# Arbol-Project/dcdf

Measured on AMD Instinct MI355X. Metric: raster cells/s encoded (Snapshot+Log build), higher is better.
Workload: dtype int32; 1 GPU; configs[2]: 4096x4096x365 i32 raster, seed 0xDCDF0003, tiled into 3072 [<=32,256,256] chunks; 3072 of them on this GPU; workload_key=config2/i32/n3072/w1, chunks_total=3072, chunks_on_rank0=3072, cells_total=6123683840, k=2, device=gfx950:sramecc+:xnack- AMD Radeon Graphics, 256 CUs, failed_tiles_rank0=0, encoded_bytes_rank0=4115239087, snapshots_rank0=3072, bytes_verified_vs_oracle=0, parallelism=chunks sharded over 1 GPU(s), no data-path collective

## Files before the change

dcdf_amd/csrc/k2r_capi_encode.hip:

```cpp
#include <algorithm>
#include <atomic>
#include <condition_variable>
#include <cstdio>
#include <cstdlib>
#include <cstring>
#include <deque>
#include <memory>
#include <mutex>
#include <new>
#include <thread>
#include <vector>

#include <sched.h>

#include <cstring>
#include <queue>

#include "k2r_launch.h"
#include "k2r_runtime.h"

using namespace k2r;

namespace k2r {

// ... 463 lines not shown
    if (std::getenv("K2R_PROFILE_PRINT")) {
        uint64_t acc[NPROF] = {0};
        for (size_t i = 0; i < n; i++)
            for (int k = 0; k < NPROF; k++) acc[k] += e->results[i].prof[k];
        uint64_t tot = 0;
        for (int k = 0; k < NPROF; k++) tot += acc[k];
        static const char* names[NPROF] = {"p1 load+analysis", "p2 top", "p3 own/top nodes", "reduce4", "clear+hdr",
                                           "emit C snapshot", "emit C/Q log", "T/eqB bitmaps", "Lmax dac | V0,M0 bitmaps", "Lmin dac | zero bitmaps",
                                           "emit pass A", "emit pass B/I", "sizes+heuristic", "winner scan", "byte-1 pass A", "fast: phase 1",
                                           "fast: wait p1", "fast: top+plan", "fast: copy-out", "fast: bitmaps"};
        for (int k = 0; k < NPROF; k++)
            std::fprintf(stderr, "k2r-prof %-18s %14llu cyc %5.1f%%\n", names[k], (unsigned long long)acc[k],
                         tot ? 100.0 * (double)acc[k] / (double)tot : 0.0);
#ifdef K2R_PROFILE
        {
            static uint64_t w[16][NPROF][2];
            std::memset(w, 0, sizeof(w));
            for (size_t i = 0; i < n; i++)
                for (int v = 0; v < 16; v++)
                    for (int k = 0; k < NPROF; k++) {
                        w[v][k][0] += e->results[i].pw[v][k][0];
                        w[v][k][1] += e->results[i].pw[v][k][1];
                    }
            int nw = 0;
            for (int v = 0; v < 16; v++) {
                uint64_t t = 0;
                for (int k = 0; k < NPROF; k++) t += w[v][k][0] + w[v][k][1];
                if (t) nw = v + 1;
            }
            uint64_t insts = 0;
            for (size_t i = 0; i < n; i++) insts += e->results[i].snapshots + e->results[i].logs;
            double all = 0;
            for (int k = 0; k < NPROF; k++)
                for (int v = 0; v < nw; v++) all += (double)(w[v][k][0] + w[v][k][1]);
            all /= nw ? nw : 1;
            std::fprintf(stderr, "k2r-pw %d waves, %llu chunk-instants, %.0f cycles per chunk-instant and wave (work + wait)\n", nw,
                         (unsigned long long)insts, insts ? all / (double)insts : 0.0);
            std::fprintf(stderr, "k2r-pw %-24s %9s %9s %9s %9s %7s   (cycles per chunk-instant)\n", "phase", "work-mean", "work-max", "work-w0",
                         "wait-mean", "share");
            for (int k = 0; k < NPROF; k++) {
                double mean = 0, mx = 0, wait = 0;
                for (int v = 0; v < nw; v++) {
                    mean += (double)w[v][k][0];
                    wait += (double)w[v][k][1];
                    mx = std::max(mx, (double)w[v][k][0]);
                }
                if (mean + wait == 0) continue;
                mean /= nw;
                wait /= nw;
                const double d = insts ? (double)insts : 1.0;
                std::fprintf(stderr, "k2r-pw %-24s %9.0f %9.0f %9.0f %9.0f %6.1f%%\n", names[k], mean / d, mx / d, (double)w[0][k][0] / d, wait / d,
                             all ? 100.0 * (mean + wait) / all : 0.0);
            }
        }
#endif
        std::vector<double> per;
        uint64_t logs = 0, stash = 0;
        for (size_t i = 0; i < n; i++) {
            uint64_t t = 0;
            for (int k = 0; k < NPROF; k++) t += e->results[i].prof[k];
            const uint32_t ni = e->results[i].snapshots + e->results[i].logs;
            if (ni) per.push_back((double)t / ni);
            logs += e->results[i].logs;
            stash += e->results[i].stash_logs;
        }
        std::sort(per.begin(), per.end());
        if (!per.empty()) {
            double sum = 0;
            for (double x : per) sum += x;
            std::fprintf(stderr, "k2r-prof cycles/instant per tile: min %.0f p50 %.0f mean %.0f p90 %.0f p99 %.0f max %.0f | logs %llu from stash %llu\n",
                         per.front(), per[per.size() / 2], sum / per.size(), per[per.size() * 9 / 10], per[per.size() * 99 / 100],
                         per.back(), (unsigned long long)logs, (unsigned long long)stash);
        }
    }
    for (size_t i = 0; i < n; i++)
        if (e->results[i].status == ST_INTERNAL) {
            const uint32_t* d = e->results[i].dbg;
            std::fprintf(stderr, "dcdf_k2r: internal guard tripped on tile %zu: guard bitmask=0x%08x (bit = kGuard* in k2r_encode.h)\n",
                         i, d[0]);
        }
    for (int pass = 0; pass < 2; pass++) {
    std::vector<std::vector<uint32_t>> again(e->classes.size());
    bool any = false, unsplit = false;
    for (size_t ci = 0; ci < e->classes.size(); ci++)
        for (uint32_t ti : e->class_tiles[ci])
            if (e->results[ti].status == ST_OUT_CAPACITY || e->results[ti].status == ST_RESPLIT) {
                if (e->results[ti].status == ST_OUT_CAPACITY) {
                    const dcdf_tile_desc& t = e->desc[ti];
                    const uint64_t cap = 6 + (uint64_t)t.instants * (1 + worst_instant_bytes((uint32_t)e->classes[ci].log2s));
                    std::unique_ptr<DevBuf> b(new DevBuf());
                    K2R_HIP(b->alloc(cap));
                    e->args[ti].out = b->as<uint8_t>();
                    e->args[ti].out_cap = cap;
                    e->retry_slots.push_back(std::move(b));
                }
                const bool was_split = e->args[ti].inst_end != 0;
                e->args[ti].inst_end = 0;
                e->args[ti].shared_flag = nullptr;
                e->args[ti].shared_cmp = nullptr;
                unsplit = unsplit || was_split;
                K2R_HIP(hipMemcpy(e->d_args.as<TileArgs>() + ti, &e->args[ti], sizeof(TileArgs), hipMemcpyHostToDevice));
                again[ci].push_back(ti);
                any = true;
            }
    if (any) {
        rc = run_classes(e, &again, nullptr);
// ... 619 lines not shown
```

dcdf_amd/csrc/k2r_encode.h:

```cpp
#pragma once
#include "k2r_exec.h"


#ifndef K2R_DIAG_SKIP
#define K2R_DIAG_SKIP 0
#endif

namespace k2r {

template <int LOG2S>
struct EncCfg {
    static_assert(LOG2S >= 3 && LOG2S <= 8, "kernel body written for sidelen 8..256 (the library dispatches 16..256)");
    static constexpr int H = LOG2S;
    static constexpr int S = 1 << LOG2S;
    static constexpr int NBLK = 1 << (2 * (LOG2S - 3));
    static constexpr int NT = NBLK;
    static constexpr int NW = NT < 64 ? 1 : NT / 64;
    static constexpr int NTOP = ((1 << (2 * (H - 2))) - 1) / 3;
    static constexpr int NTOPX = NTOP - (1 << (2 * (H - 3)));
    static constexpr int TBW = (NTOPX + 31) / 32 + 1;
    static constexpr int MAXV = ((1 << (2 * (H + 1))) - 1) / 3;
    static constexpr int MAXT = ((1 << (2 * H)) - 1) / 3;
    static constexpr int WV = (MAXV + 31) / 32;
    static constexpr int WT = (MAXT + 31) / 32;
    static constexpr int top_off(int h) { return ((1 << (2 * (H - 2))) - (1 << (2 * (H - h + 1)))) / 3; }
};

struct EncRegs {
    uint32_t d2[4];
    uint32_t flags;
    uint32_t u2;
    uint32_t sc[MAX_SCAN_FIELDS];
    uint64_t pf_lo;
    uint32_t pf_l2;
    uint32_t pa[5];
#ifdef K2R_REGCOPY
    uint32_t cw[32];
#endif
};

K2R_HD uint32_t unpackI(int h, uint64_t lo, uint64_t top) {
    switch (h) {
        case 1: return (uint32_t)(lo & 0xffffu);
        case 2: return (uint32_t)((lo >> 16) & 0x3fffu);
        case 3: return (uint32_t)((lo >> 30) & 0xfffu);
        case 4: return (uint32_t)(top & 0x3ffu);
        case 5: return (uint32_t)((top >> 10) & 0xffu);
        case 6: return (uint32_t)((top >> 18) & 0x3fu);
        case 7: return (uint32_t)((top >> 24) & 0xfu);
        case 8: return (uint32_t)((top >> 28) & 0x3u);
    }
    return 0;
}
K2R_HD uint64_t packTop(int h) {
    switch (h) {
        case 4: return 1ull;
        case 5: return 1ull << 10;
        case 6: return 1ull << 18;
        case 7: return 1ull << 24;
        case 8: return 1ull << 28;
    }
    return 0;
}

struct Cls {
    uint32_t c1 = 0, c2 = 0, c3 = 0;
    K2R_HD void add(uint32_t zz, bool on) {
        c1 += (on && zz > 0xffu) ? 1u : 0u;
        c2 += (on && zz > 0xffffu) ? 1u : 0u;
        c3 += (on && zz > 0xffffffu) ? 1u : 0u;
    }
    K2R_HD void add4(uint32_t z0, uint32_t z1, uint32_t z2, uint32_t z3, bool on) {
        if (on && ((z0 | z1 | z2 | z3) > 0xffu)) {
            add(z0, true);
            add(z1, true);
            add(z2, true);
            add(z3, true);
        }
// ... 418 lines not shown
    uint32_t offZ[C::H + 2];
    uint32_t LT, N0, M0;
    K2R_HD void from_counts(const uint32_t* ni) {
        constexpr int H = C::H;
#pragma unroll
        for (int h = 1; h <= H; h++) Ni[h] = ni[h];
        finish();
    }
    K2R_HD void from(uint64_t lo, uint64_t top) {
        constexpr int H = C::H;
#pragma unroll
        for (int h = 1; h <= H; h++) Ni[h] = unpackI(h, lo, top);
        finish();
    }
    K2R_HD void finish() {
        constexpr int H = C::H;
        Ni[H + 1] = 0;
        uint32_t v = 0, i = 0, z = 0;
#pragma unroll
        for (int h = H; h >= 0; h--) {
            uint32_t nv = (h == H) ? 1u : 4u * Ni[h + 1];
            offV[h] = v;
            offI[h] = i;
            offZ[h] = z;
            v += nv;
            if (h >= 1) {
                i += Ni[h];
                z += nv - Ni[h];
            }
        }
        N0 = v;
        LT = offV[0];
        M0 = i;
    }
};

template <class C>
struct InstPlan {
    Totals<C> T[2];
    DacLayout V[2], M[2];
    uint32_t need;
    uint32_t narrow;
    uint32_t log_size, snap_lb, eq_off;
    uint32_t as_snapshot, use_stash, isize;
    uint32_t lngV[3], lngM[3];
};

template <class C>
struct EncPool {
    static constexpr int POOL_L1 = 4 * C::NBLK;
    static constexpr int POOL_BMV1 = 12 * C::NBLK;
    static constexpr int POOL_PREFV = POOL_BMV1 + C::WV + 1;
#ifdef K2R_PROFILE
    static constexpr int POOLFILL = 1828 - 16 * NPROF * 4;
#else
    static constexpr int POOLFILL = 1828;
#endif
    static constexpr int POOLW = POOL_PREFV + C::WV + 2 + (C::H == 8 ? POOLFILL : 0);
    static constexpr int CAPI_REC = (POOLW * 53 / 100) / 5;
    static constexpr int CAPQ_REC = (POOLW - 5 * CAPI_REC) / 3;
    static constexpr int QBASE = 5 * CAPI_REC;
    static constexpr int OVI_WORDS = 5 * 4 * C::NBLK;
    static constexpr int OVQ_WORDS = 3 * 16 * C::NBLK;
};

template <class C>
struct EncShared : EncPool<C> {
    using EncPool<C>::POOL_L1;
    using EncPool<C>::POOL_BMV1;
    using EncPool<C>::POOL_PREFV;
    using EncPool<C>::POOLW;
    int32_t tmin[C::NTOP], tmax[C::NTOP], smin[C::NTOP], smax[C::NTOP], diff[C::NTOP];
    uint32_t eq[C::NTOP];
    uint32_t pool[EncPool<C>::POOLW];
    uint32_t bmT[C::WT + 1], bmE[C::WT + 1];
    uint32_t bmV0[C::WV + 1];
    uint32_t bmM[2][C::WT + 1];
    uint32_t prefM[C::WT + 2];
    uint32_t wsum[C::NW][MAX_SCAN_FIELDS];
    uint32_t tot[MAX_SCAN_FIELDS];
    K2R_HD uint32_t* L2() { return pool; }
    K2R_HD uint16_t* L1() { return (uint16_t*)(pool + POOL_L1); }
    K2R_HD uint32_t* bmV1() { return pool + POOL_BMV1; }
    K2R_HD uint32_t* prefV() { return pool + POOL_PREFV; }
    static constexpr int PREFTOP = 48;
    uint32_t prefTopV[PREFTOP + 1];
    uint32_t pfx[3][C::NBLK];
    uint32_t lq[C::NBLK][2];
    uint32_t li[C::NBLK];
    uint32_t tbS[C::TBW], tbL[C::TBW];
    uint32_t tbP[C::TBW + 1];
    uint32_t ttR[C::H + 2];
    uint32_t nlistV, nlistM;
    uint32_t stI, stQ;
    InstPlan<C> pl;
    int32_t err;
    uint32_t work;
    uint32_t fault[6];
    uint64_t prof[NPROF], prof_last;
#ifdef K2R_PROFILE
    uint64_t pw[16][NPROF][2];
#endif
};

template <class EX>
K2R_HD bool guard_ok(EX& ex, bool ok, uint32_t code, uint32_t inst, uint32_t tid, uint32_t value, uint32_t limit) {
    ex.gfail |= ok ? 0u : (1u << (code & 31u));
    (void)inst; (void)tid; (void)value; (void)limit;
    return ok;
}
template <bool UNIFORM_SPAN = true, class EX>
K2R_HD uint32_t guard_pos(EX& ex, uint32_t pos, uint32_t span, uint32_t limit, uint32_t code) {
#if defined(__HIP_DEVICE_COMPILE__) && !defined(K2R_GUARD_FULL)
    int32_t r;
    if (UNIFORM_SPAN) asm("v_med3_i32 %0, %1, 0, %2" : "=v"(r) : "v"((int32_t)pos), "s"((int32_t)limit - (int32_t)span));
    else asm("v_med3_i32 %0, %1, 0, %2" : "=v"(r) : "v"((int32_t)pos), "v"((int32_t)limit - (int32_t)span));
    (void)ex; (void)code;
    return (uint32_t)r;
#else
    const bool ok = pos + span <= limit;
    ex.gfail |= ok ? 0u : (1u << (code & 31u));
    return ok ? pos : 0u;
#endif
}
template <class EX>
K2R_HD void guard_flush(EX& ex) {
    if (ex.gfail) {
        ex.lds_or(&ex.sh.fault[0], ex.gfail);
        ex.gfail = 0;
    }
}
enum : uint32_t {
    kGuardVPos = 0, kGuardVSlot = 1, kGuardMPos = 2, kGuardMSlot = 3, kGuardTOwn = 4, kGuardEOwn = 5, kGuardTRun1 = 6,
    kGuardTRun2 = 7, kGuardE2 = 8, kGuardE1 = 9, kGuardListPos = 10, kGuardListRank = 14, kGuardList2 = 18, kGuardList1 = 19,
};

template <class EX>
K2R_HD void bm_set(EX& ex, uint32_t* bm, uint32_t p) {
    ex.lds_or(&bm[p >> 5], 0x80000000u >> (p & 31));
}
template <class EX>
K2R_HD void bm_or_run(EX& ex, uint32_t* bm, uint32_t p, uint32_t len, uint32_t bits) {
    if (len == 0 || bits == 0) return;
    const uint64_t v = (uint64_t)bits << (64 - len);
    const uint32_t sh = p & 31;
    const uint64_t w = v >> sh;
    const uint32_t hi = (uint32_t)(w >> 32), lo = (uint32_t)w;
// ... 284 lines not shown
template <class C, bool PADDED, int VEC, class EX>
K2R_HD void encode_chunk(EX& ex, const TileArgs& ta, TileResult* res, uint64_t* listV, uint64_t* listM, uint32_t* scmp, uint32_t* ovf) {
    constexpr int H = C::H;
    constexpr int NT = C::NT;
    auto& sh = ex.sh;
    using SH = EncShared<C>;
    static_assert(!(PADDED && VEC != 0), "vector loads need an unpadded tile");
    const uint32_t stash_cap = ta.stash_words != 0 ? ta.stash_words : 0xffffffffu;
    uint32_t* const ovI = ovf;
    uint32_t* const ovQ = ovf + SH::OVI_WORDS;

    uint8_t* const out = ta.out;
    const uint64_t cap = ta.out_cap;

    auto blk_origin = [&](int tid, uint32_t& r0, uint32_t& c0) {
        uint32_t br, bc;
        morton_decode((uint32_t)tid, br, bc);
        r0 = br * 8;
        c0 = bc * 8;
#if defined(__HIP_DEVICE_COMPILE__)
        asm volatile("" : "+v"(r0), "+v"(c0));
#endif
    };
    auto inval = [&](uint32_t r, uint32_t c) -> bool { return PADDED && (r >= ta.rows || c >= ta.cols); };
    auto top_inval = [&](int h, uint32_t j) -> bool {
        if (!PADDED) return false;
        uint32_t br, bc;
        morton_decode(j, br, bc);
        return inval(br << h, bc << h);
    };

    const uint32_t i_begin = ta.inst_begin, i_end = ta.inst_end != 0 ? ta.inst_end : ta.instants;
    const bool cont = i_begin > 0;
    const bool head = !cont && ta.shared_flag != nullptr;
    bool published = false;
    uint32_t* cmp = scmp;
    constexpr uint32_t NO_HDR = 0xffffffffu;
    uint32_t carry = 0;
    uint32_t off = cont ? 0u : 6u;
    uint32_t n_blocks = 0;
    uint32_t blk_hdr = cont ? NO_HDR : 6u;
    uint32_t blk_count = 0;
    uint32_t s_idx = 0;
    bool s_cmp = false;
    int32_t s_base = 0;
    uint32_t n_snap = 0, n_log = 0, n_stash = 0;
    int32_t status = ST_OK;

    ex.par([&](int tid, EncRegs&) {
        if (tid == 0) {
            sh.err = 0;
            sh.stI = 0;
            sh.stQ = 0;
            for (int i = 0; i < 6; i++) sh.fault[i] = 0;
            for (int i = 0; i < NPROF; i++) sh.prof[i] = 0;
            if (cap >= 6 && !cont) {
                out[0] = (uint8_t)ta.dtype;
                out[1] = (uint8_t)ta.fbits;
            }
        }
    });
    if (cap < 7 && !cont) status = ST_OUT_CAPACITY;
#ifdef K2R_PROFILE
    if (!EX::kSim) {
        ex.par([&](int tid, EncRegs&) {
            if (tid == 0) sh.prof_last = clock64();
            if ((tid & 63) == 0)
                for (int k = 0; k < NPROF; k++) sh.pw[tid >> 6][k][0] = sh.pw[tid >> 6][k][1] = 0;
        });
        ex.pw_start();
    }
#endif

#ifdef K2R_REGCOPY
    constexpr bool kRegCopy = !PADDED;
#else
    constexpr bool kRegCopy = false;
#endif
    [[maybe_unused]] auto lean_node = [&](uint32_t ltid, int p, uint32_t& B, uint32_t& j) {
        if (EX::kSim) {
            B = ltid;
            j = (uint32_t)p;
        } else {
            constexpr uint32_t NTW = NT < 64 ? NT : 64, BPP = NTW / 4;
            const uint32_t lane = ltid & 63u;
            B = (ltid & ~63u) + BPP * (uint32_t)p + (lane >> 2);
            j = lane & 3u;
        }
    };
    auto compact_pass = [&](uint32_t from, bool to_global) {
        if (kRegCopy) {
#ifdef K2R_REGCOPY
            ex.par_nosync([&](int tid, EncRegs& r) {
                const uint32_t ltid = opaque((uint32_t)tid);
                int32_t lerr = 0;
#pragma unroll
                for (int p = 0; p < 4; p++) {
                    uint32_t B, j, br, bc;
                    lean_node(ltid, p, B, j);
                    morton_decode(4u * B + j, br, bc);
                    int32_t t16[16];
                    load_sub16<false, VEC>(ta, from, 4u * br, 4u * bc, 0, t16, lerr);
#pragma unroll
                    for (int q = 0; q < 2; q++)
#pragma unroll
                        for (int c = 0; c < 4; c++)
// ... 684 lines not shown
        };
        auto log_vmax = [&](int h, uint32_t j) -> int32_t {
            const int a = C::top_off(h) + (int)j;
            return top_inval(h, j) ? 0 : sh.tmax[a] - sh.smax[a];
        };
        auto log_vmin = [&](int h, uint32_t j) -> int32_t {
            const int a = C::top_off(h) + (int)j;
            return sh.tmin[a] - sh.smin[a];
        };

        auto top_decode = [&](uint32_t n, int& h, uint32_t& j) {
            h = 4;
#pragma unroll
            for (int k = 4; k < H; k++)
                if (n >= (uint32_t)(C::top_off(k + 1) - C::NBLK)) h = k + 1;
            j = n - (uint32_t)(C::top_off(h) - C::NBLK);
        };
        auto tbit = [&](int h, uint32_t j) -> uint32_t { return (uint32_t)(C::top_off(h) - C::NBLK) + j; };

        ex.par_nosync([&](int tid, EncRegs& r) {
            uint32_t sI3 = 0, lI3 = 0;
            uint32_t wide = (r.flags >> 28) & 1u;
            Cls lMax, lMin;
            uint32_t sTop = 0, lTop = 0;
            auto node = [&](int h, uint32_t j) {
                if (PS(h, j)) {
                    if (h == 3) sI3 = 1;
                    else {
                        ex.lds_or(&sh.tbS[tbit(h, j) >> 5], 1u << (tbit(h, j) & 31));
                        sTop += (uint32_t)packTop(h);
                    }
                }
                if (have_s) {
                    const bool visL = (h == H) ? true : PL(h + 1, j >> 2);
                    const bool pL = PL(h, j);
                    const int32_t vx = log_vmax(h, j), vn = log_vmin(h, j);
                    lMax.add1(vx, visL);
                    lMin.add1(vn, pL);
                    wide |= ((visL && (vx < -32768 || vx > 32767)) || (pL && (vn < -32768 || vn > 32767))) ? 1u : 0u;
                    if (pL) {
                        if (h == 3) lI3 = 1;
                        else {
                            ex.lds_or(&sh.tbL[tbit(h, j) >> 5], 1u << (tbit(h, j) & 31));
                            lTop += (uint32_t)packTop(h);
                        }
                    }
                }
            };
            const uint32_t wt = opaque((uint32_t)tid);
            node(3, wt);
            if (tid == 0) {
                sh.stI = 0;
                sh.stQ = 0;
            }
            if (wt < (uint32_t)C::NTOPX) {
                int h;
                uint32_t j;
                top_decode(wt, h, j);
                node(h, j);
            }
            r.sc[1] = sI3 | (lI3 << 16);
            r.sc[2] = sTop;
            r.sc[4] = lTop;
            r.sc[5] = lMax.c1 | (lMin.c1 << 16);
            r.sc[6] = wide;
            uint32_t cL0 = 0, cL1 = 0, mL1 = 0, cL2 = 0, mL2 = 0;
            if (have_s) {
                const uint32_t fl = sh.li[tid];
                cL0 = popc32(sh.lq[tid][0]) + popc32(sh.lq[tid][1]);
                cL1 = popc32(fl & 0x0f0f0f0fu);
                mL1 = popc32(fl & 0xf0f0f0f0u);
#pragma unroll
                for (int j = 0; j < 4; j++) {
                    const int32_t vx = rec16(r.d2[j] & 0xffffu), vn = rec16(r.d2[j] >> 16);
                    r.d2[j] = ((uint32_t)vx & 0xffffu) | ((uint32_t)vn << 16);
                    const bool P2L = ((r.u2 >> j) & 1u) == 0 && ((r.flags >> j) & 1u) == 0;
                    cL2 += lI3 ? lng(vx) : 0u;
                    mL2 += P2L ? lng(vn) : 0u;
                }
            }
            r.sc[7] = cL0;
            r.sc[8] = cL1 | (cL2 << 16);
            r.sc[9] = mL1 | (mL2 << 16);
        });
        ex.stamp(2);
        ex.template scan_begin<10>();
        ex.stamp(3);

        auto classes_pass = [&](const int which) {
#ifdef K2R_SIM_TRACE
            if (EX::kSim) __builtin_printf("classes_pass(%d) inst=%u\n", which, inst);
#endif
            ex.par_nosync([&](int tid, EncRegs& r) {
                uint32_t r0, c0;
                blk_origin(tid, r0, c0);
                int32_t lerr = 0;
                Cls vMax, vMin;
                auto cnode = [&](int h, uint32_t j) {
                    if (which == 0) {
                        vMax.add(zz32(snap_vmax(h, j)), (h == H) ? true : PS(h + 1, j >> 2));
                        vMin.add(zz32(snap_vmin(h, j)), PS(h, j));
                    } else {
                        vMax.add(zz32(log_vmax(h, j)), (h == H) ? true : PL(h + 1, j >> 2));
                        vMin.add(zz32(log_vmin(h, j)), PL(h, j));
                    }
                };
// ... 205 lines not shown
        }
        if (need & 2u) {
            classes_pass(0);
            plan(3);
        }
        const bool as_snapshot = ex.uni(sh.pl.as_snapshot) != 0;
        const bool use_stash = ex.uni(sh.pl.use_stash) != 0;
        const uint32_t isize = ex.uni(sh.pl.isize);
        const uint32_t log_eq_off = ex.uni(sh.pl.eq_off);
        const Totals<C>& TT = sh.pl.T[as_snapshot ? 0 : 1];
        const DacLayout& DV = sh.pl.V[as_snapshot ? 0 : 1];
        const DacLayout& DM = sh.pl.M[as_snapshot ? 0 : 1];

        uint32_t hdr_patch_off = 0, hdr_patch_val = 0;
        bool do_patch = false;
        if (as_snapshot) {
            if (have_s) {
                if (blk_hdr == NO_HDR) carry = blk_count;
                else {
                    do_patch = true;
                    hdr_patch_off = blk_hdr;
                    hdr_patch_val = blk_count;
                }
                n_blocks++;
            }
            blk_hdr = off;
            off += 1;
            blk_count = 0;
            s_idx = inst;
            n_snap++;
            const int32_t rmin = ex.uni(sh.tmin[C::top_off(H)]), rmax = ex.uni(sh.tmax[C::top_off(H)]);
            s_cmp = (int64_t)rmax - (int64_t)rmin <= 65535 && inst + 1 < ta.instants;
            s_base = rmin;
            cmp = (head && inst == 0) ? ta.shared_cmp : scmp;
        } else {
            n_log++;
        }
        if ((uint64_t)off + isize > cap) {
            status = ST_OUT_CAPACITY;
            break;
        }
        uint8_t* const io = out + off;
        n_stash += use_stash ? 1u : 0u;
        ex.stamp(12);
        ex.par([&](int tid, EncRegs& r) {
            const uint32_t pI12 = as_snapshot ? r.sc[0] : r.sc[3];
            const uint32_t pI3 = as_snapshot ? (r.sc[1] & 0xffffu) : (r.sc[1] >> 16);
            const uint32_t pL0 = r.sc[7], pL12 = r.sc[8], pM12 = r.sc[9];
            r.pf_lo = (uint64_t)pI12 | ((uint64_t)pI3 << 30);
            r.pf_l2 = (pL12 >> 16) | (pM12 & 0xffff0000u);
            sh.pfx[0][tid] = pI12;
            sh.pfx[1][tid] = pL0;
            sh.pfx[2][tid] = (pL12 & 0xffffu) | (pM12 << 16);
            if (tid <= C::TBW) {
                const uint32_t* const tbw = as_snapshot ? sh.tbS : sh.tbL;
                uint32_t run = 0;
                for (int w = 0; w < tid && w < C::TBW; w++) run += popc32(tbw[w]);
                sh.tbP[tid] = run;
            }
            if (tid == 0) {
                sh.nlistV = 0;
                sh.nlistM = 0;
                if (do_patch) out[hdr_patch_off] = (uint8_t)hdr_patch_val;
                io[0] = 2;
                store_be32(io + 1, ta.rows);
                store_be32(io + 5, ta.cols);
                store_be32(io + 9, (uint32_t)C::S);
                io[DV.bm_off[0] - 1] = (uint8_t)DV.nlev;
                io[DM.bm_off[0] - 1] = (uint8_t)DM.nlev;
                if (ta.minmax) {
                    ta.minmax[2 * inst] = sh.tmin[C::top_off(H)];
                    ta.minmax[2 * inst + 1] = sh.tmax[C::top_off(H)];
                }
            }
        });

        ex.stamp(4);
        const uint32_t nlevV = ex.uni(DV.nlev), nlevM = ex.uni(DM.nlev);
        const DacSink sinkV{io + ex.uni(DV.by_off[0]), sh.bmV0, listV, &sh.nlistV, ex.uni(DV.n[0]), ex.uni(DV.n[1]), inst, kGuardVPos,
                            io + ex.uni(DV.by_off[1]), use_stash ? sh.prefTopV : sh.prefV()};
        const DacSink sinkM{io + ex.uni(DM.by_off[0]), sh.bmM[0], listM, &sh.nlistM, ex.uni(DM.n[0]), ex.uni(DM.n[1]), inst, kGuardMPos,
                            io + ex.uni(DM.by_off[1]), sh.prefM};

        const bool snap_dyn = as_snapshot;
        const Totals<C>& TT_dyn = TT;
        auto passA = [&](auto mode_tag) {
          constexpr int MODE = decltype(mode_tag)::value;
          ex.par_nosync([&](int tid, EncRegs& r) {
            uint32_t r0, c0;
            blk_origin(tid, r0, c0);
            const uint64_t pLo = r.pf_lo;

            const bool as_snapshot = MODE == EM_P0 ? false : snap_dyn;
            const Totals<C>& TT = MODE == EM_P0 ? sh.pl.T[1] : TT_dyn;
            const uint32_t* const tb = as_snapshot ? sh.tbS : sh.tbL;
            if (MODE == EM_P0) r.pa[2] = 0;
            constexpr int GMODE = (MODE == EM_P0) ? (int)EM_ONE : MODE;
            auto enode = [&](int h, uint32_t j, const int slot) {
                const bool vis = (h == H) ? true : bit_test(tb, tbit(h + 1, j >> 2));
                if (!vis) return;
                const bool p = (h == 3) ? (as_snapshot ? PS(3, j) : PL(3, j)) : bit_test(tb, tbit(h, j));
                auto trank = [&](uint32_t b) -> uint32_t {
                    return sh.tbP[b >> 5] + popc32(tb[b >> 5] & ((1u << (b & 31u)) - 1u));
                };
                uint32_t vrank = 0;
                if (h < H) vrank = 4 * (trank(tbit(h + 1, j >> 2)) - sh.ttR[h + 1]) + (j & 3);
                const uint32_t idx = TT.offV[h] + vrank;
                const uint32_t irank = (h == 3) ? unpackI(3, pLo, 0) : trank(tbit(h, j)) - sh.ttR[h];
                const uint32_t zv = zz32(as_snapshot ? snap_vmax(h, j) : log_vmax(h, j));
                emit_val<0, MODE>(ex, sinkV, idx, zv, tid);
                if (MODE == EM_P0) {
                    r.pa[3 * slot] = idx;
                    r.pa[2] |= (zv >> 8) << (16 * slot);
                }
                if (p) {
                    bm_set(ex, sh.bmT, guard_pos(ex, idx, 1, TT.LT, kGuardTOwn));
                    const uint32_t zm = zz32(as_snapshot ? snap_vmin(h, j) : log_vmin(h, j));
                    emit_val<1, MODE>(ex, sinkM, TT.offI[h] + irank, zm, tid);
                    if (MODE == EM_P0) {
                        r.pa[3 * slot + 1] = TT.offI[h] + irank;
                        r.pa[2] |= (zm >> 8) << (16 * slot + 8);
                    }
// ... 82 lines not shown
                                smx2 = s16[i] > smx2 ? s16[i] : smx2;
                            }
                            vx = inv2 ? 0 : mx2 - smx2;
                            vn = mn2 - smn2;
                        }
                    } else {
                        vx = (int32_t)(int16_t)(r.d2[j] & 0xffffu);
                        vn = (int32_t)r.d2[j] >> 16;
                    }
                    if (as_snapshot) {
                        P2[j] = !unif2;
                        z2v[j] = zz32(vx);
                        zm2[j] = zz32(vn);
                    } else {
                        P2[j] = !unif2 && ((r.flags >> j) & 1u) == 0;
                        z2v[j] = zz32(vx);
                        zm2[j] = zz32(vn);
                        if (!P2[j]) {
                            erun = (erun << 1) | (unif2 ? 0u : 1u);
                            elen++;
                        }
                    }
                    tb2 = (tb2 << 1) | (P2[j] ? 1u : 0u);
                }
                emit4<0, GMODE>(ex, sinkV, p2, z2v[0], z2v[1], z2v[2], z2v[3], tid, sh.pl.lngV[2] + (r.pf_l2 & 0xffffu));
                bm_or_run(ex, sh.bmT, guard_pos(ex, p2, 4, TT.LT, kGuardTRun2), 4, tb2);
                if (!as_snapshot) bm_or_run(ex, sh.bmE, guard_pos<false>(ex, TT.offZ[2] + 4 * E3 - E2, elen, TT.LT - TT.M0, kGuardE2), elen, erun);
                uint32_t n2 = 0, pre = E1, lm = sh.pl.lngM[2] + (r.pf_l2 >> 16);
                const uint32_t cshift = as_snapshot ? 4u : 16u;
#pragma unroll
                for (int j = 0; j < 4; j++) {
                    if (P2[j]) {
                        emit_val<1, GMODE>(ex, sinkM, TT.offI[2] + E2 + n2, zm2[j], tid, lm);
                        lm += zm2[j] > 0xffu ? 1u : 0u;
                        if (MODE == EM_LIST)
                            sh.L2()[guard_pos(ex, E2 + n2, 1, 4 * C::NBLK, kGuardList2)] = ((uint32_t)tid << 2) | (uint32_t)j | (pre << 12);
                        n2++;
                        pre += (r.flags >> (cshift + 3 * j)) & 7u;
                    }
                }
            }
            guard_flush(ex);
        });
        };
        const uint32_t nI2 = ex.uni(TT.Ni[2]), nI1 = ex.uni(TT.Ni[1]);
        if (use_stash) {
            if (!(K2R_DIAG_SKIP & 1)) passA(EmTag<EM_P0>{});
            ex.stamp(10);
            auto passI = [&](auto ovf_tag) {
              constexpr bool OVF = decltype(ovf_tag)::value != 0;
              ex.par_nosync([&](int tid, EncRegs&) {
                const uint32_t offV1 = TT.offV[1], offZ1 = TT.offZ[1], offI1 = TT.offI[1], lt = TT.LT, ne = TT.LT - TT.M0;
                const uint32_t lv1 = sh.pl.lngV[1], lm1 = sh.pl.lngM[1];
                for (uint32_t k = (uint32_t)tid; k < nI2; k += NT) {
                    uint32_t rec[5];
                    if (!OVF || k < (uint32_t)SH::CAPI_REC) {
#pragma unroll
                        for (int i = 0; i < 5; i++) rec[i] = sh.pool[5u * k + i];
                    } else {
                        gload_words<5>(ovI + 5u * (k - (uint32_t)SH::CAPI_REC), rec);
                    }
                    const uint32_t hdr = rec[0];
                    const uint32_t own = hdr & 1023u;
                    const uint32_t pf = sh.pfx[0][own], pl = sh.pfx[2][own];
                    const uint32_t kk = ((pf >> 16) & 0x3fffu) + ((hdr >> 10) & 3u);
                    const uint32_t pre = (pf & 0xffffu) + ((hdr >> 12) & 15u);
                    const uint32_t tb1 = (hdr >> 16) & 15u, e4 = (hdr >> 20) & 15u, elen = 4u - popc32(tb1);
                    uint32_t erun = 0;
#pragma unroll
                    for (int qq = 0; qq < 4; qq++) {
                        const uint32_t t0 = ((tb1 >> (3 - qq)) & 1u) ^ 1u;
                        erun = (erun << t0) | ((e4 >> (3 - qq)) & t0);
                    }
                    const uint32_t below = sh.li[own] & ((1u << (8u * ((hdr >> 10) & 3u))) - 1u);
                    uint32_t w[4];
#pragma unroll
                    for (int qq = 0; qq < 4; qq++) w[qq] = rec[1 + qq];
                    const uint32_t p1 = offV1 + 4 * kk;
                    emit4<0, EM_ONE>(ex, sinkV, p1, zz32(rec16(w[0] & 0xffffu)), zz32(rec16(w[1] & 0xffffu)),
                                     zz32(rec16(w[2] & 0xffffu)), zz32(rec16(w[3] & 0xffffu)), tid,
                                     lv1 + (pl & 0xffffu) + popc32(below & 0x0f0f0f0fu));
                    bm_or_run(ex, sh.bmT, guard_pos(ex, p1, 4, lt, kGuardTRun1), 4, tb1);
                    bm_or_run(ex, sh.bmE, guard_pos<false>(ex, offZ1 + 4 * kk - pre, elen, ne, kGuardE1), elen, erun);
                    uint32_t n1 = 0, lm = lm1 + (pl >> 16) + popc32(below & 0xf0f0f0f0u);
#pragma unroll
                    for (int qq = 0; qq < 4; qq++) {
                        if ((tb1 >> (3 - qq)) & 1u) {
                            const uint32_t zm = zz32(rec16(w[qq] >> 16));
                            emit_val<1, EM_ONE>(ex, sinkM, offI1 + pre + n1, zm, tid, lm);
                            lm += zm > 0xffu ? 1u : 0u;
                            n1++;
                        }
                    }
                }
                guard_flush(ex);
              });
            };
            if (K2R_DIAG_SKIP & 2) {
            } else if (rec_ovf) passI(EmTag<1>{});
            else passI(EmTag<0>{});
            ex.stamp(11);
            auto passQ = [&](auto ovf_tag) {
              constexpr bool OVF = decltype(ovf_tag)::value != 0;
              ex.par([&](int tid, EncRegs&) {
                const uint32_t offV0 = TT.offV[0], lv0 = sh.pl.lngV[0];
                for (uint32_t m = (uint32_t)tid; m < nI1; m += NT) {
                    uint32_t q[3];
                    if (!OVF || m < (uint32_t)SH::CAPQ_REC) {
#pragma unroll
                        for (int i = 0; i < 3; i++) q[i] = sh.pool[SH::QBASE + 3u * m + i];
                    } else {
                        gload_words<3>(ovQ + 3u * (m - (uint32_t)SH::CAPQ_REC), q);
                    }
                    const uint32_t hdr = q[0], a = q[1], b = q[2];
                    const uint32_t own = hdr & 1023u;
                    const uint32_t ord = (hdr >> 10) & 15u;
                    const uint32_t pos = (sh.pfx[0][own] & 0xffffu) + ord;
                    const uint32_t f0 = sh.lq[own][0], f1 = sh.lq[own][1], cut = (1u << (4u * (ord & 7u))) - 1u;
                    const uint32_t before = ord < 8u ? popc32(f0 & cut) : popc32(f0) + popc32(f1 & cut);
                    emit4<0, EM_ONE>(ex, sinkV, offV0 + 4 * pos, zz32(rec16(a & 0xffffu)), zz32(rec16(a >> 16)),
                                     zz32(rec16(b & 0xffffu)), zz32(rec16(b >> 16)), tid, lv0 + sh.pfx[1][own] + before);
                }
                guard_flush(ex);
              });
            };
            if (K2R_DIAG_SKIP & 4) ex.barrier();
            else if (rec_ovf) passQ(EmTag<1>{});
            else passQ(EmTag<0>{});
            ex.stamp(6);
            {
                const uint32_t lt = ex.uni(TT.LT), m0 = ex.uni(TT.M0);
                const BmJob jobs[4] = {{sh.bmT, lt, nullptr, 0, io + 13},
                                       {sh.bmE, lt - m0, nullptr, 0, io + log_eq_off},
                                       {sh.bmV0, sinkV.n0, sh.prefTopV, SH::PREFTOP, nlevV > 0 ? io + ex.uni(DV.bm_off[0]) : nullptr},
                                       {sh.bmM[0], sinkM.n0, sh.prefM, SH::PREFTOP, nlevM > 0 ? io + ex.uni(DM.bm_off[0]) : nullptr}};
                if (!(K2R_DIAG_SKIP & 8)) bitmaps_finish<C, 4>(ex, jobs);
            }
            ex.stamp(8);
            if (nlevV > 1 || nlevM > 1) {
                if (!(K2R_DIAG_SKIP & 16)) ex.par_nosync([&](int tid, EncRegs& r) {
                    auto put = [&](const DacSink& d, uint32_t* bm0, uint32_t pos, uint32_t hi) {
                        if (hi) {
                            pos = guard_pos(ex, pos, 1, d.n0 < 32u * SH::PREFTOP ? d.n0 : 32u * SH::PREFTOP, d.code);
                            gstore8(d.plane1 + guard_pos(ex, bm_rank(bm0, d.pref, pos), 1, d.n1, d.code + 1), (uint8_t)hi);
                        }
                    };
                    const uint32_t hb = r.pa[2];
                    put(sinkV, sh.bmV0, r.pa[0], hb & 0xffu);
                    put(sinkM, sh.bmM[0], r.pa[1], (hb >> 8) & 0xffu);
                    put(sinkV, sh.bmV0, r.pa[3], (hb >> 16) & 0xffu);
                    put(sinkM, sh.bmM[0], r.pa[4], hb >> 24);
                    guard_flush(ex);
                });
                ex.stamp(14);
                if (nlevV > 1 && !(K2R_DIAG_SKIP & 32)) bitmap_write_zero<C>(ex, sinkV.n1, io + ex.uni(DV.bm_off[1]));
                if (nlevM > 1 && !(K2R_DIAG_SKIP & 32)) bitmap_write_zero<C>(ex, sinkM.n1, io + ex.uni(DM.bm_off[1]));
            }
            ex.stamp(9);
        } else {
// ... 175 lines not shown
```

dcdf_amd/csrc/k2r_exec.h:

```cpp
#pragma once
#include "k2r_common.h"

namespace k2r {

constexpr int MAX_SCAN_FIELDS = 16;

#if defined(__HIPCC__)

template <class SH, class TR, int NT>
struct GpuExec {
    SH& sh;
    TR r;
    const int tid;
    uint32_t gfail = 0;
    static constexpr int kNT = NT;
    static constexpr bool kSim = false;

    __device__ GpuExec(SH& s) : sh(s), tid((int)threadIdx.x) {}

#ifdef K2R_PROFILE
    uint64_t pw_last = 0, pw_work = 0, pw_wait = 0;
    __device__ __forceinline__ void pw_before() {
        const uint64_t t = __builtin_amdgcn_s_memtime();
        pw_work += t - pw_last;
        pw_last = t;
    }
    __device__ __forceinline__ void pw_after() {
        const uint64_t t = __builtin_amdgcn_s_memtime();
        pw_wait += t - pw_last;
        pw_last = t;
    }
    __device__ __forceinline__ void pw_start() { pw_last = __builtin_amdgcn_s_memtime(); pw_work = pw_wait = 0; }
#else
    __device__ __forceinline__ void pw_before() {}
    __device__ __forceinline__ void pw_after() {}
    __device__ __forceinline__ void pw_start() {}
#endif

    __device__ __forceinline__ void lds_barrier() {
        pw_before();
        asm volatile("s_waitcnt lgkmcnt(0)\n\ts_barrier" ::: "memory");
        pw_after();
    }
    __device__ __forceinline__ void wave_lds_fence() { asm volatile("s_waitcnt lgkmcnt(0)" ::: "memory"); }
    __device__ __forceinline__ void barrier_global() {
        pw_before();
        __syncthreads();
        pw_after();
    }

    __device__ __forceinline__ void publish(uint32_t* flag, uint32_t value, uint32_t payload) {
        __syncthreads();
        if (tid == 0) {
            __hip_atomic_store(flag + 1, payload, __ATOMIC_RELAXED, __HIP_MEMORY_SCOPE_AGENT);
            __builtin_amdgcn_fence(__ATOMIC_RELEASE, "agent");
            __hip_atomic_store(flag, value, __ATOMIC_RELAXED, __HIP_MEMORY_SCOPE_AGENT);
        }
    }
    __device__ __forceinline__ uint32_t await(const uint32_t* flag, uint32_t timeout_value) {
        if (tid == 0) {
            uint32_t v = 0;
            for (uint32_t spin = 0; spin < (1u << 22); spin++) {
                v = __hip_atomic_load(flag, __ATOMIC_RELAXED, __HIP_MEMORY_SCOPE_AGENT);
                if (v != 0) break;
                __builtin_amdgcn_s_sleep(32);
            }
            __builtin_amdgcn_fence(__ATOMIC_ACQUIRE, "agent");
            sh.err = v != 0 ? (int32_t)v : (int32_t)timeout_value;
        }
        __syncthreads();
        const uint32_t v = (uint32_t)__builtin_amdgcn_readfirstlane(sh.err);
// ... 168 lines not shown
    }
    __device__ __forceinline__ static int32_t row_min_of_quads(int32_t x) {
        int32_t y = (int32_t)row_ror<4>((uint32_t)x);
        x = x < y ? x : y;
        y = (int32_t)row_ror<8>((uint32_t)x);
        return x < y ? x : y;
    }
    __device__ __forceinline__ static int32_t row_max_of_quads(int32_t x) {
        int32_t y = (int32_t)row_ror<4>((uint32_t)x);
        x = x > y ? x : y;
        y = (int32_t)row_ror<8>((uint32_t)x);
        return x > y ? x : y;
    }
    __device__ __forceinline__ static uint32_t row_or_of_quads(uint32_t x) {
        x |= row_ror<4>(x);
        return x | row_ror<8>(x);
    }
    __device__ __forceinline__ static int32_t wave_min_of_rows(int32_t x) {
        const int32_t a = __builtin_amdgcn_readlane(x, 0), b = __builtin_amdgcn_readlane(x, 16), c = __builtin_amdgcn_readlane(x, 32),
                      d = __builtin_amdgcn_readlane(x, 48);
        const int32_t p = a < b ? a : b, q = c < d ? c : d;
        return p < q ? p : q;
    }
    __device__ __forceinline__ static int32_t wave_max_of_rows(int32_t x) {
        const int32_t a = __builtin_amdgcn_readlane(x, 0), b = __builtin_amdgcn_readlane(x, 16), c = __builtin_amdgcn_readlane(x, 32),
                      d = __builtin_amdgcn_readlane(x, 48);
        const int32_t p = a > b ? a : b, q = c > d ? c : d;
        return p > q ? p : q;
    }
    __device__ __forceinline__ static uint32_t wave_or_of_rows(uint32_t x) {
        return (uint32_t)(__builtin_amdgcn_readlane((int)x, 0) | __builtin_amdgcn_readlane((int)x, 16) | __builtin_amdgcn_readlane((int)x, 32) |
                          __builtin_amdgcn_readlane((int)x, 48));
    }
    __device__ __forceinline__ static uint32_t lane_pull(uint32_t src, uint32_t v) {
        return (uint32_t)__builtin_amdgcn_ds_bpermute((int)(src << 2), (int)v);
    }

    __device__ __forceinline__ void stash_alloc(uint32_t c, uint32_t* cntA, uint32_t* cntB, uint32_t& a, uint32_t& b, uint32_t& enda,
                                                uint32_t& endb) {
        constexpr int W = NT < 64 ? NT : 64;
        const int lane = tid & 63;
        const uint32_t incl = wave_incl_scan(c);
        const uint32_t tot = (uint32_t)__builtin_amdgcn_readlane((int)incl, W - 1);
        uint32_t ret = 0;
        if (lane < 2) ret = atomicAdd(lane == 0 ? cntA : cntB, lane == 0 ? (tot & 0xffffu) : (tot >> 16));
        const uint32_t ba = (uint32_t)__builtin_amdgcn_readlane((int)ret, 0), bb = (uint32_t)__builtin_amdgcn_readlane((int)ret, W > 1 ? 1 : 0);
        const uint32_t excl = incl - c;
        a = ba + (excl & 0xffffu);
        b = bb + (excl >> 16);
        enda = ba + (tot & 0xffffu);
        endb = bb + (tot >> 16);
    }

    __device__ __forceinline__ uint32_t lds_or_nr(uint32_t* p, uint32_t v) { atomicOr(p, v); return 0; }
    __device__ __forceinline__ uint32_t lds_or(uint32_t* p, uint32_t v) { return atomicOr(p, v); }
    __device__ __forceinline__ uint32_t lds_add(uint32_t* p, uint32_t v) { return atomicAdd(p, v); }
    __device__ __forceinline__ int32_t lds_min(int32_t* p, int32_t v) { return atomicMin(p, v); }

    template <int NF, bool TOT = true>
    __device__ __forceinline__ void scan() {
        constexpr int W = NT < 64 ? NT : 64;
        constexpr int NW = NT < 64 ? 1 : NT / 64;
        const int lane = tid & 63;
        const int wave = __builtin_amdgcn_readfirstlane(tid >> 6);
        int incl[NF];
#pragma unroll
        for (int f = 0; f < NF; f++) incl[f] = (int)r.sc[f];
        wave_incl_scan_n(incl);
        if (lane == W - 1) {
#pragma unroll
            for (int f = 0; f < NF; f++) sh.wsum[wave][f] = (uint32_t)incl[f];
        }
        lds_barrier();
        int x[NF];
#pragma unroll
        for (int f = 0; f < NF; f++) x[f] = (lane < NW) ? (int)sh.wsum[lane < NW ? lane : 0][f] : 0;
        row_incl_scan_n(x);
#pragma unroll
        for (int f = 0; f < NF; f++) {
            const uint32_t tot = (uint32_t)__builtin_amdgcn_readlane(x[f], NW - 1);
            const uint32_t base = wave == 0 ? 0u : (uint32_t)__builtin_amdgcn_readlane(x[f], wave - 1);
            r.sc[f] = base + (uint32_t)incl[f] - r.sc[f];
            if (TOT && tid == 0) sh.tot[f] = tot;
        }
        if (TOT) lds_barrier();
    }
};

#endif

#if !defined(__HIP_DEVICE_COMPILE__)
}
#include <vector>
namespace k2r {

template <class SH, class TR, int NT>
struct SimExec {
    SH& sh;
    std::vector<TR> regs;
    uint32_t gfail = 0;
    static constexpr int kNT = NT;
    static constexpr bool kSim = true;

    explicit SimExec(SH& s) : sh(s), regs(NT) {}

    template <class F>
    void par(F&& f) {
        for (int t = 0; t < NT; t++) f(t, regs[t]);
    }
    template <class F>
    void par_nosync(F&& f) {
        for (int t = 0; t < NT; t++) f(t, regs[t]);
    }
    void barrier() {}
    void wave_lds_fence() {}
    void barrier_global() {}
    void publish(uint32_t* flag, uint32_t value, uint32_t payload) {
        flag[1] = payload;
        flag[0] = value;
    }
    uint32_t await(const uint32_t* flag, uint32_t timeout_value) { return flag[0] != 0 ? flag[0] : timeout_value; }
    uint32_t flag_payload(const uint32_t* flag) { return flag[1]; }
    void stamp(int) {}
    template <class T>
    T uni(T v) const { return v; }
    template <int NF, int F0 = 0>
    void reduce() {
        for (int f = F0; f < F0 + NF; f++) {
            uint32_t run = 0;
            for (int t = 0; t < NT; t++) run += regs[t].sc[f];
            sh.tot[f] = run;
        }
    }

    template <int NF>
    void scan_begin() {
        scan<NF, true>();
    }
    static constexpr int planner() { return 0; }
    uint32_t lane_value(uint32_t v, int) const { return v; }
    template <int NF>
    void scan_finish(uint32_t (&t)[NF]) {
        for (int f = 0; f < NF; f++) t[f] = sh.tot[f];
    }


    void stash_alloc(uint32_t c, uint32_t* cntA, uint32_t* cntB, uint32_t& a, uint32_t& b, uint32_t& enda, uint32_t& endb) {
        a = *cntA;
        b = *cntB;
        *cntA += c & 0xffffu;
        *cntB += c >> 16;
        enda = *cntA;
        endb = *cntB;
    }
    uint32_t lds_or_nr(uint32_t* p, uint32_t v) {
        *p |= v;
        return 0;
    }
    uint32_t lds_or(uint32_t* p, uint32_t v) {
        uint32_t o = *p;
        *p = o | v;
        return o;
    }
    uint32_t lds_add(uint32_t* p, uint32_t v) {
        uint32_t o = *p;
        *p = o + v;
        return o;
    }
    int32_t lds_min(int32_t* p, int32_t v) {
        int32_t o = *p;
        if (v < o) *p = v;
        return o;
    }

    template <int NF, bool TOT = true>
    void scan() {
        for (int f = 0; f < NF; f++) {
            uint32_t run = 0;
            for (int t = 0; t < NT; t++) {
                const uint32_t v = regs[t].sc[f];
                regs[t].sc[f] = run;
                run += v;
            }
            sh.tot[f] = run;
        }
    }
};
#endif

}
```

Measured before the change: 552.4 billion cells/s.

## Balance per-wave work with dynamic record claiming and rotated single-thread tasks

Replaces the static strided loops over I and Q records with wave-granular dynamic work claiming through an LDS atomic counter, so waves that finish early pick up more records. Moves the single-thread tbP prefix and header writes onto threads in different waves chosen by a rotation, and computes the tbP prefix sequentially in one thread instead of one thread per word. It also adds per-wave profiling tables to the host report. The atomic claiming adds one LDS atomic per wave iteration, and the pool shrinks by two words to make room for the counters.

```diff
diff --git a/dcdf_amd/csrc/k2r_capi_encode.hip b/dcdf_amd/csrc/k2r_capi_encode.hip
--- a/dcdf_amd/csrc/k2r_capi_encode.hip
+++ b/dcdf_amd/csrc/k2r_capi_encode.hip
@@ -539,6 +539,45 @@
                 std::fprintf(stderr, "k2r-pw %-24s %9.0f %9.0f %9.0f %9.0f %6.1f%%\n", names[k], mean / d, mx / d, (double)w[0][k][0] / d, wait / d,
                              all ? 100.0 * (mean + wait) / all : 0.0);
             }
+            const double d = insts ? (double)insts : 1.0;
+            for (int c = 0; c < 2; c++) {
+                std::fprintf(stderr, "k2r-pw-%s %-24s", c ? "wait" : "work", "phase \\ wave");
+                for (int v = 0; v < nw; v++) std::fprintf(stderr, " %6d", v);
+                std::fprintf(stderr, "\n");
+                for (int k = 0; k < NPROF; k++) {
+                    uint64_t any = 0;
+                    for (int v = 0; v < nw; v++) any += w[v][k][0] + w[v][k][1];
+                    if (!any) continue;
+                    std::fprintf(stderr, "k2r-pw-%s %-24s", c ? "wait" : "work", names[k]);
+                    for (int v = 0; v < nw; v++) std::fprintf(stderr, " %6.0f", (double)w[v][k][c] / d);
+                    std::fprintf(stderr, "\n");
+                }
+            }
+            static const struct { const char* name; int n; int k[3]; } groups[] = {
+                {"A + I + Q records", 3, {10, 11, 6}}, {"replay + zero bm + p1", 3, {14, 9, 0}}, {"p3 + scan", 2, {2, 3}},
+                {"p2 top", 1, {1}}, {"sizes+heuristic", 1, {12}}, {"clear+hdr", 1, {4}}, {"V0,M0 bitmaps", 1, {8}},
+                {"emit C snapshot", 1, {5}}, {"T/eqB bitmaps", 1, {7}}};
+            std::fprintf(stderr, "k2r-pw-group %-24s", "group \\ wave");
+            for (int v = 0; v < nw; v++) std::fprintf(stderr, " %6d", v);
+            std::fprintf(stderr, " %7s %7s\n", "max", "mean");
+            double crit = 0, avg = 0;
+            for (const auto& g : groups) {
+                double mx = 0, mean = 0;
+                std::fprintf(stderr, "k2r-pw-group %-24s", g.name);
+                for (int v = 0; v < nw; v++) {
+                    double s = 0;
+                    for (int i = 0; i < g.n; i++) s += (double)w[v][g.k[i]][0];
+                    std::fprintf(stderr, " %6.0f", s / d);
+                    mx = std::max(mx, s);
+                    mean += s;
+                }
+                mean /= nw ? nw : 1;
+                std::fprintf(stderr, " %7.0f %7.0f\n", mx / d, mean / d);
+                crit += mx;
+                avg += mean;
+            }
+            std::fprintf(stderr, "k2r-pw-group sum of the group maxima %.0f, of the group means %.0f, imbalance %.0f (cycles per chunk-instant)\n",
+                         crit / d, avg / d, (crit - avg) / d);
         }
 #endif
         std::vector<double> per;
diff --git a/dcdf_amd/csrc/k2r_encode.h b/dcdf_amd/csrc/k2r_encode.h
--- a/dcdf_amd/csrc/k2r_encode.h
+++ b/dcdf_amd/csrc/k2r_encode.h
@@ -24,6 +24,8 @@
     static constexpr int WV = (MAXV + 31) / 32;
     static constexpr int WT = (MAXT + 31) / 32;
     static constexpr int top_off(int h) { return ((1 << (2 * (H - 2))) - (1 << (2 * (H - h + 1)))) / 3; }
+    static constexpr int kWaveHeader = 1;
+    static constexpr int kWavePrefix = 2;
 };
 
 struct EncRegs {
@@ -548,9 +550,9 @@
     static constexpr int POOL_BMV1 = 12 * C::NBLK;
     static constexpr int POOL_PREFV = POOL_BMV1 + C::WV + 1;
 #ifdef K2R_PROFILE
-    static constexpr int POOLFILL = 1828 - 16 * NPROF * 4;
-#else
-    static constexpr int POOLFILL = 1828;
+    static constexpr int POOLFILL = 1826 - 16 * NPROF * 4;
+#else
+    static constexpr int POOLFILL = 1826;
 #endif
     static constexpr int POOLW = POOL_PREFV + C::WV + 2 + (C::H == 8 ? POOLFILL : 0);
     static constexpr int CAPI_REC = (POOLW * 53 / 100) / 5;
@@ -589,6 +591,7 @@
     uint32_t ttR[C::H + 2];
     uint32_t nlistV, nlistM;
     uint32_t stI, stQ;
+    uint32_t tkI, tkQ;
     InstPlan<C> pl;
     int32_t err;
     uint32_t work;
@@ -979,6 +982,8 @@
             sh.err = 0;
             sh.stI = 0;
             sh.stQ = 0;
+            sh.tkI = 0;
+            sh.tkQ = 0;
             for (int i = 0; i < 6; i++) sh.fault[i] = 0;
             for (int i = 0; i < NPROF; i++) sh.prof[i] = 0;
             if (cap >= 6 && !cont) {
@@ -1769,6 +1774,8 @@
             if (tid == 0) {
                 sh.stI = 0;
                 sh.stQ = 0;
+                sh.tkI = 0;
+                sh.tkQ = 0;
             }
             if (wt < (uint32_t)C::NTOPX) {
                 int h;
@@ -2080,22 +2087,29 @@
             sh.pfx[0][tid] = pI12;
             sh.pfx[1][tid] = pL0;
             sh.pfx[2][tid] = (pL12 & 0xffffu) | (pM12 << 16);
-            if (tid <= C::TBW) {
+            const uint32_t tp = EX::item(tid, C::kWavePrefix), th = EX::item(tid, C::kWaveHeader);
+            if (tp == 0) {
                 const uint32_t* const tbw = as_snapshot ? sh.tbS : sh.tbL;
-                uint32_t run = 0;
-                for (int w = 0; w < tid && w < C::TBW; w++) run += popc32(tbw[w]);
-                sh.tbP[tid] = run;
-            }
-            if (tid == 0) {
+                uint32_t wd[C::TBW], run = 0;
+#pragma unroll
+                for (int w = 0; w < C::TBW; w++) wd[w] = tbw[w];
+#pragma unroll
+                for (int w = 0; w < C::TBW; w++) {
+                    sh.tbP[w] = run;
+                    run += popc32(wd[w]);
+                }
+                sh.tbP[C::TBW] = run;
+            }
+            if (th == 0) {
                 sh.nlistV = 0;
                 sh.nlistM = 0;
-                if (do_patch) out[hdr_patch_off] = (uint8_t)hdr_patch_val;
-                io[0] = 2;
-                store_be32(io + 1, ta.rows);
-                store_be32(io + 5, ta.cols);
-                store_be32(io + 9, (uint32_t)C::S);
-                io[DV.bm_off[0] - 1] = (uint8_t)DV.nlev;
-                io[DM.bm_off[0] - 1] = (uint8_t)DM.nlev;
+                if (do_patch) gstore8(out + hdr_patch_off, (uint8_t)hdr_patch_val);
+                gstore8(io, 2);
+                gstore32u(io + 1, __builtin_bswap32(ta.rows));
+                gstore32u(io + 5, __builtin_bswap32(ta.cols));
+                gstore32u(io + 9, __builtin_bswap32((uint32_t)C::S));
+                gstore8(io + DV.bm_off[0] - 1, (uint8_t)DV.nlev);
+                gstore8(io + DM.bm_off[0] - 1, (uint8_t)DM.nlev);
                 if (ta.minmax) {
                     ta.minmax[2 * inst] = sh.tmin[C::top_off(H)];
                     ta.minmax[2 * inst + 1] = sh.tmax[C::top_off(H)];
@@ -2284,7 +2298,7 @@
               ex.par_nosync([&](int tid, EncRegs&) {
                 const uint32_t offV1 = TT.offV[1], offZ1 = TT.offZ[1], offI1 = TT.offI[1], lt = TT.LT, ne = TT.LT - TT.M0;
                 const uint32_t lv1 = sh.pl.lngV[1], lm1 = sh.pl.lngM[1];
-                for (uint32_t k = (uint32_t)tid; k < nI2; k += NT) {
+                for (uint32_t k = ex.take(&sh.tkI, tid); k < nI2; k = ex.take(&sh.tkI, tid)) {
                     uint32_t rec[5];
                     if (!OVF || k < (uint32_t)SH::CAPI_REC) {
 #pragma unroll
@@ -2336,7 +2350,7 @@
               constexpr bool OVF = decltype(ovf_tag)::value != 0;
               ex.par([&](int tid, EncRegs&) {
                 const uint32_t offV0 = TT.offV[0], lv0 = sh.pl.lngV[0];
-                for (uint32_t m = (uint32_t)tid; m < nI1; m += NT) {
+                for (uint32_t m = ex.take(&sh.tkQ, tid); m < nI1; m = ex.take(&sh.tkQ, tid)) {
                     uint32_t q[3];
                     if (!OVF || m < (uint32_t)SH::CAPQ_REC) {
 #pragma unroll
diff --git a/dcdf_amd/csrc/k2r_exec.h b/dcdf_amd/csrc/k2r_exec.h
--- a/dcdf_amd/csrc/k2r_exec.h
+++ b/dcdf_amd/csrc/k2r_exec.h
@@ -4,6 +4,17 @@
 namespace k2r {
 
 constexpr int MAX_SCAN_FIELDS = 16;
+
+template <int NT>
+K2R_HD constexpr uint32_t wave_item(int tid, int rot) {
+    constexpr uint32_t NW = NT <= 64 ? 1u : (uint32_t)NT / 64u;
+    return NT <= 64 ? (uint32_t)tid : ((((uint32_t)tid >> 6) + (uint32_t)rot) % NW) * 64u + ((uint32_t)tid & 63u);
+}
+template <int NT>
+K2R_HD constexpr int wave_rot_to(int v) {
+    constexpr int NW = NT <= 64 ? 1 : NT / 64;
+    return (NW - v % NW) % NW;
+}
 
 #if defined(__HIPCC__)
 
@@ -17,6 +28,7 @@
     static constexpr bool kSim = false;
 
     __device__ GpuExec(SH& s) : sh(s), tid((int)threadIdx.x) {}
+    __device__ __forceinline__ static uint32_t item(int t, int first) { return wave_item<NT>(t, wave_rot_to<NT>(first)); }
 
 #ifdef K2R_PROFILE
     uint64_t pw_last = 0, pw_work = 0, pw_wait = 0;
@@ -291,6 +303,13 @@
         endb = bb + (tot >> 16);
     }
 
+    __device__ __forceinline__ uint32_t take(uint32_t* ctr, int t) {
+        constexpr uint32_t W = NT < 64 ? NT : 64;
+        uint32_t first = 0;
+        if ((t & 63) == 0) first = atomicAdd(ctr, W);
+        return (uint32_t)__builtin_amdgcn_readfirstlane((int)first) + (uint32_t)(t & 63);
+    }
+
     __device__ __forceinline__ uint32_t lds_or_nr(uint32_t* p, uint32_t v) { atomicOr(p, v); return 0; }
     __device__ __forceinline__ uint32_t lds_or(uint32_t* p, uint32_t v) { return atomicOr(p, v); }
     __device__ __forceinline__ uint32_t lds_add(uint32_t* p, uint32_t v) { return atomicAdd(p, v); }
@@ -342,6 +361,7 @@
     static constexpr bool kSim = true;
 
     explicit SimExec(SH& s) : sh(s), regs(NT) {}
+    static uint32_t item(int t, int first) { return wave_item<NT>(t, wave_rot_to<NT>(first)); }
 
     template <class F>
     void par(F&& f) {
@@ -392,6 +412,7 @@
         enda = *cntA;
         endb = *cntB;
     }
+    uint32_t take(uint32_t* ctr, int) { return (*ctr)++; }
     uint32_t lds_or_nr(uint32_t* p, uint32_t v) {
         *p |= v;
         return 0;
```

Result: faster. 564.7 billion cells/s (median of 6 runs) (+2.2%).
